# KwonGihyun/TweedieMix

Hardware: AMD Instinct MI355X
Metric: denoise steps/sec @ SDXL 1024^2 K=3 concepts (fusion phase); images/sec at 1/2/4/8 GPUs (higher is better)
Workload: dtype bf16

## Files before the change

tweediemix_amd/csrc/attention.hip:

```cpp
#include "common.h"
#include <type_traits>
#include <stdlib.h>

namespace {

#ifndef TMIX_ATTN_ABL
#define TMIX_ATTN_ABL 0
#endif
constexpr int AABL = TMIX_ATTN_ABL;

typedef __attribute__((ext_vector_type(8))) __bf16 frag_ab;
typedef __attribute__((ext_vector_type(2))) __bf16 bf16x2_t;

constexpr int QB = 128;
constexpr int KB = 64;
constexpr int TILE = KB * 64 * 2;
constexpr int STAGE = 2 * TILE;

struct AttnParams {
    const bf16_t* Q; int64_t ldq, strideQ;
    const bf16_t* K; int64_t ldk, strideK;
    const bf16_t* Vt; int64_t ldvt, strideVt;
    bf16_t* O; int64_t ldo, strideO;
    int B, H, Sq, Skv, nq;
    float scale_log2e;
    unsigned long long* prof; int prof_detail;
    unsigned char* O8; int64_t ldo8; unsigned char* Sc; int64_t ldSc;
    int n_full, lsplit, tpp; float* ws; unsigned* tickets;
};

__device__ __forceinline__ void glds16(const void* gsrc, char* lds_dst) {
    __builtin_amdgcn_global_load_lds((const __attribute__((address_space(1))) void*)gsrc,
                                     (__attribute__((address_space(3))) void*)lds_dst, 16, 0, 0);
}

template <int N> __device__ __forceinline__ void wait_vmcnt() { asm volatile("s_waitcnt vmcnt(%0)" ::"n"(N) : "memory"); }

__device__ __forceinline__ float xor16_max(float x) {
    auto r = __builtin_amdgcn_permlane16_swap(__float_as_uint(x), __float_as_uint(x), false, false);
    return fmaxf(__uint_as_float(r[0]), __uint_as_float(r[1]));
}
__device__ __forceinline__ float xor32_max(float x) {
    auto r = __builtin_amdgcn_permlane32_swap(__float_as_uint(x), __float_as_uint(x), false, false);
    return fmaxf(__uint_as_float(r[0]), __uint_as_float(r[1]));
}
__device__ __forceinline__ float xor16_sum(float x) {
    auto r = __builtin_amdgcn_permlane16_swap(__float_as_uint(x), __float_as_uint(x), false, false);
    return __uint_as_float(r[0]) + __uint_as_float(r[1]);
}
__device__ __forceinline__ float xor32_sum(float x) {
    auto r = __builtin_amdgcn_permlane32_swap(__float_as_uint(x), __float_as_uint(x), false, false);
    return __uint_as_float(r[0]) + __uint_as_float(r[1]);
}

__device__ __forceinline__ void store_row_f8(const AttnParams& p, int64_t row, int h, int fg, const float (&v)[4][4], bool ok) {
#pragma unroll
    for (int blk = 0; blk < 2; ++blk) {
        float f[8], am = 0.f;
#pragma unroll
        for (int k = 0; k < 8; ++k) {
            f[k] = (float)(__bf16)v[2 * blk + (k >> 2)][k & 3];
            am = fmaxf(am, fabsf(f[k]));
        }
        am = xor16_max(am); am = xor32_max(am);
        const int e = e8m0_for_amax(am);
        const float inv = exp2_neg_int(e);
        int q0 = __builtin_amdgcn_cvt_pk_fp8_f32(f[0] * inv, f[1] * inv, 0, false); q0 = __builtin_amdgcn_cvt_pk_fp8_f32(f[2] * inv, f[3] * inv, q0, true);
        int q1 = __builtin_amdgcn_cvt_pk_fp8_f32(f[4] * inv, f[5] * inv, 0, false); q1 = __builtin_amdgcn_cvt_pk_fp8_f32(f[6] * inv, f[7] * inv, q1, true);
        if (ok) {
            unsigned char* dst = p.O8 + row * p.ldo8 + h * 64 + blk * 32 + fg * 4;
            *(int*)dst = q0; *(int*)(dst + 16) = q1;
            if (fg == 0) p.Sc[(int64_t)(h * 2 + blk) * p.ldSc + row] = (unsigned char)(e + 127);
        }
    }
}

constexpr int SPLIT_MAX = 4;
constexpr int SPLIT_VEC = 9;
__device__ __forceinline__ void st_coherent(f32x4* dst, f32x4 v) { asm volatile("global_store_dwordx4 %0, %1, off sc1" :: "v"(dst), "v"(v) : "memory"); }
__device__ __forceinline__ f32x4 ld_coherent(const f32x4* src) { f32x4 v; asm volatile("global_load_dwordx4 %0, %1, off sc1" : "=v"(v) : "v"(src) : "memory"); return v; }

__device__ __forceinline__ uint32_t pk_bf16(float a, float b) {
    bf16x2_t v = {(__bf16)a, (__bf16)b};
    return *(uint32_t*)&v;
}

constexpr int NSP = 4;
constexpr int SMEM_P = NSP * STAGE;

__global__ void __launch_bounds__(256, 2) attn_fwd_pipe_kernel(const AttnParams p) {
#ifndef TMIX_NO_KERNARG_TOUCH
    kernarg_touch<(int)sizeof(AttnParams)>();
#endif
    constexpr int LOADS = 4;
    constexpr int NR = 2;
    extern __shared__ __attribute__((aligned(16))) char smem[];
    const int tid = threadIdx.x, lane = tid & 63;
    const int w = __builtin_amdgcn_readfirstlane(tid >> 6);
    const int fr = lane & 15, fg = lane >> 4;
    const bool prof_on = p.prof != nullptr && tid == 0;
    unsigned long long pt0 = 0, pt1 = 0, pt2 = 0;
    if (prof_on) pt0 = prof_enter(p.prof, blockIdx.x == 0, p.prof_detail);

    int bid, part = 0;
    if ((int)blockIdx.x < p.n_full) bid = xcd_remap(blockIdx.x, p.n_full);
    else {
        const int j = (int)blockIdx.x - p.n_full, k = j >> 3, n_tail8 = ((int)gridDim.x - p.n_full) >> (3 + p.lsplit);
        bid = p.n_full + (j & 7) * n_tail8 + (k >> p.lsplit);
        part = k & ((1 << p.lsplit) - 1);
    }
    const bool split = (int)blockIdx.x >= p.n_full;
    const int bh = bid / p.nq, qt = bid - bh * p.nq;
    const int b = bh / p.H, h = bh - b * p.H;
    const int q0 = qt * QB + w * 32;
    const int key0 = split ? part * p.tpp * KB : 0;
    const int skv = split ? p.tpp * KB : p.Skv;
    const bf16_t* Qb = p.Q + (int64_t)b * p.strideQ + h * 64;
    const bf16_t* Kb = p.K + (int64_t)b * p.strideK + h * 64 + (int64_t)key0 * p.ldk;
    const bf16_t* Vb = p.Vt + (int64_t)b * p.strideVt + (int64_t)h * 64 * p.ldvt + key0;

    const int lrow = lane >> 3;
    const int schunk = ((lane & 7) ^ lrow) * 8;
    int krow[NR], voff[NR];
    const int ldk = (int)p.ldk, ldvt = (int)p.ldvt;
#pragma unroll
    for (int r = 0; r < NR; ++r) {
        const int rho = (r * 4 + w) * 8 + lrow;
        const int f = rho >> 4, i = rho & 15;
        krow[r] = 32 * (f >> 1) + 8 * (i >> 2) + 4 * (f & 1) + (i & 3);
        voff[r] = rho * ldvt;
    }
    const int nt = (skv + KB - 1) / KB;
    const int vlim = ldvt - 8 - key0;
    auto stage = [&](int t) {
        char* sK = smem + (t & (NSP - 1)) * STAGE;
        char* sV = sK + TILE;
        const int kv0 = t * KB;
        int c = kv0 + schunk; if (c > vlim) c = vlim;
#pragma unroll
        for (int r = 0; r < NR; ++r) {
            const int off = (r * 4 + w) * 1024;
            int key = kv0 + krow[r]; if (key > skv - 1) key = skv - 1;
            glds16(Kb + (unsigned)(key * ldk + schunk), sK + off);
            glds16(Vb + (unsigned)(voff[r] + c), sV + off);
        }
    };
#pragma unroll
    for (int t = 0; t < NSP - 1; ++t)
        if (t < nt) stage(t);

    frag_ab qf[2][2];
#pragma unroll
    for (int qi = 0; qi < 2; ++qi) {
        int q = q0 + qi * 16 + fr; if (q > p.Sq - 1) q = p.Sq - 1;
#pragma unroll
        for (int ds = 0; ds < 2; ++ds) {
            const frag_ab raw = *(const frag_ab*)(Qb + (int64_t)q * p.ldq + ds * 32 + fg * 8);
#pragma unroll
            for (int j = 0; j < 8; ++j) qf[qi][ds][j] = (__bf16)((float)raw[j] * p.scale_log2e);
        }
    }

    f32x4 o[4][2];
#pragma unroll
    for (int i = 0; i < 4; ++i) { o[i][0] = (f32x4){0.f, 0.f, 0.f, 0.f}; o[i][1] = (f32x4){0.f, 0.f, 0.f, 0.f}; }
    constexpr float THR = 8.0f;
    f32x4 negm[2] = {{0.f, 0.f, 0.f, 0.f}, {0.f, 0.f, 0.f, 0.f}};
    f32x4 lacc[2] = {{0.f, 0.f, 0.f, 0.f}, {0.f, 0.f, 0.f, 0.f}};
    frag_ab ones;
#pragma unroll
    for (int j = 0; j < 8; ++j) ones[j] = (__bf16)1.0f;
    bool first = true;

    frag_ab kf[2][4];
    frag_ab vf[2][4];
    uint32_t pb[2][2][4];
    const int swk0 = ((0 * 4 + fg) ^ (fr & 7)) << 4, swk1 = ((1 * 4 + fg) ^ (fr & 7)) << 4;
    auto read_k = [&](int t) {
        const char* sK = smem + (t & (NSP - 1)) * STAGE;
#pragma unroll
        for (int f = 0; f < 4; ++f) kf[0][f] = *(const frag_ab*)(sK + (f * 16 + fr) * 128 + swk0);
    };

    auto half1 = [&](int t, f32x4 (&sc)[4][2], f32x4 (&sp)[4][2], auto cur_tag, auto prev_tag) {
        constexpr bool CUR = decltype(cur_tag)::value, PREV = decltype(prev_tag)::value;
        const char* sV = smem + ((t - 1) & (NSP - 1)) * STAGE + TILE;
        const char* sKc = smem + (t & (NSP - 1)) * STAGE;
#pragma unroll
        for (int n = 0; n < 16; ++n) {
            const int dh = n >> 3, f = (n >> 1) & 3, qi = n & 1;
            if constexpr (CUR) {
                if constexpr (AABL & 4) { if (dh == 0) sc[f][qi] = negm[qi]; asm volatile("" :: "v"(kf[dh][f])); }
                else sc[f][qi] = __builtin_amdgcn_mfma_f32_16x16x32_bf16(kf[dh][f], qf[qi][dh], dh ? sc[f][qi] : negm[qi], 0, 0, 0);
            }
// ... 110 lines not shown
    } else {
        half1(nt, sB, sA, F_{}, T_{});
        asm volatile("s_waitcnt lgkmcnt(0)" ::: "memory");
        half2(nt, sB, F_{}, T_{}, F_{});
    }

    if (prof_on) pt2 = prof_now();
    if (split) {
        const int nparts = 1 << p.lsplit, itail = bid - p.n_full;
        f32x4* wsb = (f32x4*)p.ws + ((int64_t)(itail * nparts) * 4 + w) * (SPLIT_VEC * 64) + lane;
        {
            f32x4* dst = wsb + (int64_t)part * 4 * (SPLIT_VEC * 64);
#pragma unroll
            for (int i = 0; i < 8; ++i) st_coherent(dst + i * 64, o[i >> 1][i & 1]);
            st_coherent(dst + 8 * 64, (f32x4){negm[0][0], negm[1][0], lacc[0][0], lacc[1][0]});
        }
        asm volatile("s_waitcnt vmcnt(0)" ::: "memory");
        __syncthreads();
        unsigned* flag = (unsigned*)smem;
        if (tid == 0) {
            const unsigned old = __hip_atomic_fetch_add(p.tickets + itail, 1u, __ATOMIC_RELAXED, __HIP_MEMORY_SCOPE_AGENT);
            const bool last = old == (unsigned)(nparts - 1);
            if (last) __hip_atomic_store(p.tickets + itail, 0u, __ATOMIC_RELAXED, __HIP_MEMORY_SCOPE_AGENT);
            *flag = last;
        }
        __syncthreads();
        if (!*flag) { if (prof_on) prof_leave(p.prof, p.prof_detail, pt0, pt1, pt2); return; }
        f32x4 st[SPLIT_MAX];
#pragma unroll
        for (int r = 0; r < SPLIT_MAX; ++r) if (r < nparts) st[r] = ld_coherent(wsb + (int64_t)r * 4 * (SPLIT_VEC * 64) + 8 * 64);
        asm volatile("s_waitcnt vmcnt(0)" ::: "memory");
        float m0 = -INFINITY, m1 = -INFINITY;
#pragma unroll
        for (int r = 0; r < SPLIT_MAX; ++r) if (r < nparts) { asm volatile("" : "+v"(st[r])); m0 = fmaxf(m0, -st[r][0]); m1 = fmaxf(m1, -st[r][1]); }
#pragma unroll
        for (int i = 0; i < 4; ++i) { o[i][0] = (f32x4){0.f, 0.f, 0.f, 0.f}; o[i][1] = (f32x4){0.f, 0.f, 0.f, 0.f}; }
        float l0 = 0.f, l1 = 0.f;
#pragma unroll
        for (int r = 0; r < SPLIT_MAX; ++r) {
            if (r >= nparts) break;
            f32x4 v[8];
#pragma unroll
            for (int i = 0; i < 8; ++i) v[i] = ld_coherent(wsb + (int64_t)r * 4 * (SPLIT_VEC * 64) + i * 64);
            asm volatile("s_waitcnt vmcnt(0)" ::: "memory");
            const float w0 = __builtin_amdgcn_exp2f(-st[r][0] - m0), w1 = __builtin_amdgcn_exp2f(-st[r][1] - m1);
#pragma unroll
            for (int i = 0; i < 8; ++i) { asm volatile("" : "+v"(v[i])); o[i >> 1][i & 1] += v[i] * ((i & 1) ? w1 : w0); }
            l0 += st[r][2] * w0; l1 += st[r][3] * w1;
        }
        lacc[0][0] = l0; lacc[1][0] = l1;
    }
    if (p.O8) {
#pragma unroll
        for (int qi = 0; qi < 2; ++qi) {
            const int q = q0 + qi * 16 + fr;
            const float inv = 1.0f / lacc[qi][0];
            float v[4][4];
#pragma unroll
            for (int df = 0; df < 4; ++df)
#pragma unroll
                for (int r = 0; r < 4; ++r) v[df][r] = o[df][qi][r] * inv;
            store_row_f8(p, (int64_t)b * p.Sq + min(q, p.Sq - 1), h, fg, v, q < p.Sq);
        }
        if (prof_on) prof_leave(p.prof, p.prof_detail, pt0, pt1, pt2);
        return;
    }
    bf16_t* Ob = p.O + (int64_t)b * p.strideO + h * 64;
#pragma unroll
    for (int qi = 0; qi < 2; ++qi) {
        const int q = q0 + qi * 16 + fr;
        if (q >= p.Sq) continue;
        const float inv = 1.0f / lacc[qi][0];
#pragma unroll
        for (int df = 0; df < 4; ++df) {
            uint2 v;
            v.x = pk_bf16(o[df][qi][0] * inv, o[df][qi][1] * inv);
            v.y = pk_bf16(o[df][qi][2] * inv, o[df][qi][3] * inv);
            *(uint2*)(Ob + (int64_t)q * p.ldo + df * 16 + fg * 4) = v;
        }
    }
    if (prof_on) prof_leave(p.prof, p.prof_detail, pt0, pt1, pt2);
}

constexpr int SK_MAX = 96;
constexpr int SQW = 64;

__global__ void __launch_bounds__(320, 2) attn_small_kernel(const AttnParams p) {
#ifndef TMIX_NO_KERNARG_TOUCH
    kernarg_touch<(int)sizeof(AttnParams)>();
#endif
    const int tid = threadIdx.x, lane = tid & 63;
    const int w = __builtin_amdgcn_readfirstlane(tid >> 6);
    const int fr = lane & 15, fg = lane >> 4;
    const bool prof_on = p.prof != nullptr && tid == 0;
    unsigned long long pt0 = 0, pt1 = 0;
    if (prof_on) pt0 = prof_enter(p.prof, blockIdx.x == 0, p.prof_detail);
    const int bid = xcd_remap(blockIdx.x, gridDim.x);
    const int gw = bid * (int)(blockDim.x >> 6) + w;
    const int bh = gw / p.nq, qt = gw - bh * p.nq;
    const int b = bh / p.H, h = bh - b * p.H;
    const int q0 = qt * SQW;
    if (b >= p.B) {
        if (prof_on) prof_leave(p.prof, p.prof_detail, pt0, pt0, pt0);
        return;
    }
    const bf16_t* Qb = p.Q + (int64_t)b * p.strideQ + h * 64;
    const bf16_t* Kb = p.K + (int64_t)b * p.strideK + h * 64;
    const bf16_t* Vb = p.Vt + (int64_t)b * p.strideVt + (int64_t)h * 64 * p.ldvt;
    bf16_t* Ob = p.O + (int64_t)b * p.strideO + h * 64;
    const int ldvt = (int)p.ldvt;

    frag_ab kf[6][2], vf[3][4];
#pragma unroll
    for (int f = 0; f < 6; ++f) {
        int key = 32 * (f >> 1) + 8 * (fr >> 2) + 4 * (f & 1) + (fr & 3); if (key > p.Skv - 1) key = p.Skv - 1;
#pragma unroll
        for (int ds = 0; ds < 2; ++ds) kf[f][ds] = *(const frag_ab*)(Kb + (int64_t)key * p.ldk + ds * 32 + fg * 8);
    }
#pragma unroll
    for (int ps = 0; ps < 3; ++ps) {
        int c = 32 * ps + fg * 8; if (c > ldvt - 8) c = ldvt - 8;
#pragma unroll
        for (int df = 0; df < 4; ++df) vf[ps][df] = *(const frag_ab*)(Vb + (df * 16 + fr) * ldvt + c);
    }
    frag_ab ones;
#pragma unroll
    for (int j = 0; j < 8; ++j) ones[j] = (__bf16)1.0f;
    frag_ab qraw[SQW / 32][2][2];
#pragma unroll
    for (int blk = 0; blk < SQW / 32; ++blk)
#pragma unroll
        for (int qi = 0; qi < 2; ++qi) {
            int q = q0 + blk * 32 + qi * 16 + fr; if (q > p.Sq - 1) q = p.Sq - 1;
#pragma unroll
            for (int ds = 0; ds < 2; ++ds) qraw[blk][qi][ds] = *(const frag_ab*)(Qb + (int64_t)q * p.ldq + ds * 32 + fg * 8);
        }
    if (prof_on) pt1 = prof_now();

#pragma unroll
    for (int blk = 0; blk < SQW / 32; ++blk) {
        const int qb = q0 + blk * 32;
        if (qb >= p.Sq) break;
        frag_ab qf[2][2];
#pragma unroll
        for (int qi = 0; qi < 2; ++qi) {
#pragma unroll
            for (int ds = 0; ds < 2; ++ds) {
                const frag_ab raw = qraw[blk][qi][ds];
#pragma unroll
                for (int j = 0; j < 8; ++j) qf[qi][ds][j] = (__bf16)((float)raw[j] * p.scale_log2e);
            }
        }
        f32x4 s[6][2];
        const f32x4 zero = {0.f, 0.f, 0.f, 0.f};
#pragma unroll
        for (int f = 0; f < 6; ++f)
#pragma unroll
            for (int qi = 0; qi < 2; ++qi) {
                s[f][qi] = __builtin_amdgcn_mfma_f32_16x16x32_bf16(kf[f][0], qf[qi][0], zero, 0, 0, 0);
                s[f][qi] = __builtin_amdgcn_mfma_f32_16x16x32_bf16(kf[f][1], qf[qi][1], s[f][qi], 0, 0, 0);
            }
        uint32_t pb[2][3][4];
        f32x4 o[4][2], lacc[2];
#pragma unroll
        for (int qi = 0; qi < 2; ++qi) {
            float m = -INFINITY;
#pragma unroll
            for (int f = 0; f < 6; ++f)
#pragma unroll
                for (int r = 0; r < 4; ++r) {
                    if (32 * (f >> 1) + 8 * fg + 4 * (f & 1) + r >= p.Skv) s[f][qi][r] = -INFINITY;
                    m = fmaxf(m, s[f][qi][r]);
                }
            m = xor32_max(xor16_max(m));
#pragma unroll
            for (int f = 0; f < 6; ++f)
#pragma unroll
                for (int r = 0; r < 4; ++r) s[f][qi][r] = __builtin_amdgcn_exp2f(s[f][qi][r] - m);
#pragma unroll
            for (int ps = 0; ps < 3; ++ps) {
                pb[qi][ps][0] = pk_bf16(s[2 * ps][qi][0], s[2 * ps][qi][1]);
                pb[qi][ps][1] = pk_bf16(s[2 * ps][qi][2], s[2 * ps][qi][3]);
                pb[qi][ps][2] = pk_bf16(s[2 * ps + 1][qi][0], s[2 * ps + 1][qi][1]);
                pb[qi][ps][3] = pk_bf16(s[2 * ps + 1][qi][2], s[2 * ps + 1][qi][3]);
            }
            lacc[qi] = zero;
#pragma unroll
            for (int df = 0; df < 4; ++df) o[df][qi] = zero;
        }
#pragma unroll
        for (int ps = 0; ps < 3; ++ps) {
            frag_ab p0, p1;
            __builtin_memcpy(&p0, pb[0][ps], 16);
            __builtin_memcpy(&p1, pb[1][ps], 16);
            lacc[0] = __builtin_amdgcn_mfma_f32_16x16x32_bf16(ones, p0, lacc[0], 0, 0, 0);
            lacc[1] = __builtin_amdgcn_mfma_f32_16x16x32_bf16(ones, p1, lacc[1], 0, 0, 0);
#pragma unroll
            for (int df = 0; df < 4; ++df) {
                o[df][0] = __builtin_amdgcn_mfma_f32_16x16x32_bf16(vf[ps][df], p0, o[df][0], 0, 0, 0);
                o[df][1] = __builtin_amdgcn_mfma_f32_16x16x32_bf16(vf[ps][df], p1, o[df][1], 0, 0, 0);
            }
        }
#pragma unroll
        for (int qi = 0; qi < 2; ++qi) {
            const int q = qb + qi * 16 + fr;
            const float inv = 1.0f / lacc[qi][0];
            if (p.O8) {
                float v[4][4];
#pragma unroll
                for (int df = 0; df < 4; ++df)
#pragma unroll
                    for (int r = 0; r < 4; ++r) v[df][r] = o[df][qi][r] * inv;
                store_row_f8(p, (int64_t)b * p.Sq + min(q, p.Sq - 1), h, fg, v, q < p.Sq);
                continue;
            }
            if (q >= p.Sq) continue;
#pragma unroll
            for (int df = 0; df < 4; ++df) {
                uint2 v;
                v.x = pk_bf16(o[df][qi][0] * inv, o[df][qi][1] * inv);
                v.y = pk_bf16(o[df][qi][2] * inv, o[df][qi][3] * inv);
                *(uint2*)(Ob + (int64_t)q * p.ldo + df * 16 + fg * 4) = v;
            }
        }
    }
    if (prof_on) prof_leave(p.prof, p.prof_detail, pt0, pt1, pt1);
}

}

struct AttnSplit { int n_full, lsplit, tpp, n_tail; int64_t ws_bytes; };
static bool attn_split_device_ok() {
    static int ok = -1;
    if (ok < 0) {
        int dev = 0; hipDeviceProp_t prop;
        ok = (hipGetDevice(&dev) == hipSuccess && hipGetDeviceProperties(&prop, dev) == hipSuccess && prop.multiProcessorCount * 2 == 512) ? 1 : 0;
    }
    return ok == 1;
}
static bool attn_split_plan(int B, int H, int Sq, int Skv, AttnSplit& sp) {
    constexpr int SLOTS = 512, TICKET_BYTES = 4096;
    if (Skv <= SK_MAX || (Skv % KB) || tmix_env(TMIX_ENV_ATTN_NO_SPLIT)) return false;
    const int64_t items = (int64_t)((Sq + QB - 1) / QB) * B * H;
    const int nt = Skv / KB;
    const int r = (int)(items % SLOTS);
    if (items <= SLOTS || r == 0 || (r & 7) || (SLOTS % r)) return false;
    int split = SLOTS / r, lsplit = 0;
    if (split > SPLIT_MAX) split = SPLIT_MAX;
    while ((1 << lsplit) < split) ++lsplit;
    if ((1 << lsplit) != split || (nt % split) || nt / split < 2 || r > TICKET_BYTES / 4) return false;
    sp.n_full = (int)(items - r); sp.lsplit = lsplit; sp.tpp = nt / split; sp.n_tail = r;
    sp.ws_bytes = TICKET_BYTES + (int64_t)r * split * 4 * SPLIT_VEC * 64 * 16;
    return true;
}

extern "C" int64_t tmix_attn_split_ws_bytes(int B, int H, int Sq, int Skv) {
    AttnSplit sp;
    if (B <= 0 || H <= 0 || Sq <= 0 || Skv <= 0) return 0;
    return attn_split_plan(B, H, Sq, Skv, sp) ? sp.ws_bytes : 0;
}

static int attn_entry(const void* Q, int64_t ldq, int64_t strideQ, const void* K, int64_t ldk, int64_t strideK,
                      const void* Vt, int64_t ldvt, int64_t strideVt, void* O, int64_t ldo, int64_t strideO,
                      void* O8, int64_t ldo8, void* Sc, int64_t ldSc,
                      int B, int H, int Sq, int Skv, float scale, void* stream, void* ws = nullptr, int64_t ws_bytes = 0) {
    if (!Q || !K || !Vt || (!O && !O8)) TMIX_FAIL(TMIX_EINVAL, "attn: null pointer");
    if (O8) {
        if (!Sc || (ldo8 % 4) || ldo8 < (int64_t)H * 64 || ldSc < (int64_t)B * Sq || (((uintptr_t)O8) & 3))
            TMIX_FAIL(TMIX_EINVAL, "attn_f8: needs the scale array [H*2][ldSc >= B*Sq] and 4-byte aligned e4m3 rows of ldo8 >= H*64 bytes");
        O = (void*)Q; ldo = 4; strideO = 4;
    }
    if (B <= 0 || H <= 0 || Sq <= 0 || Skv <= 0) TMIX_FAIL(TMIX_ESHAPE, "attn: empty problem B=%d H=%d Sq=%d Skv=%d", B, H, Sq, Skv);
    if ((int64_t)Skv * ldk >= (1ll << 31) || 64 * ldvt >= (1ll << 31)) TMIX_FAIL(TMIX_ESHAPE, "attn: per-head K/V extent exceeds 32-bit offsets");
    if ((ldq % 8) || (ldk % 8) || (ldvt % 8) || (ldo % 4) || (strideQ % 8) || (strideK % 8) || (strideVt % 8) || (strideO % 4))
        TMIX_FAIL(TMIX_EALIGN, "attn: leading dims / strides must keep 16-byte (Q,K,Vt) / 8-byte (O) alignment");
    if (ldvt < ((Skv + 7) / 8) * 8) TMIX_FAIL(TMIX_ESHAPE, "attn: ldvt=%lld < Skv rounded up to 8", (long long)ldvt);
    if (!aligned16(Q) || !aligned16(K) || !aligned16(Vt) || (((uintptr_t)O) & 7)) TMIX_FAIL(TMIX_EALIGN, "attn: pointer alignment");
    static bool attr_set = false;
    if (!attr_set) {
        hipError_t e = hipFuncSetAttribute((const void*)attn_fwd_pipe_kernel, hipFuncAttributeMaxDynamicSharedMemorySize, SMEM_P);
        if (e != hipSuccess) TMIX_FAIL((int)e, "hipFuncSetAttribute: %s", hipGetErrorString(e));
        attr_set = true;
    }
    AttnParams p;
    p.Q = (const bf16_t*)Q; p.ldq = ldq; p.strideQ = strideQ;
    p.K = (const bf16_t*)K; p.ldk = ldk; p.strideK = strideK;
    p.Vt = (const bf16_t*)Vt; p.ldvt = ldvt; p.strideVt = strideVt;
    p.O = (bf16_t*)O; p.ldo = ldo; p.strideO = strideO;
    p.O8 = (unsigned char*)O8; p.ldo8 = ldo8; p.Sc = (unsigned char*)Sc; p.ldSc = ldSc;
    p.B = B; p.H = H; p.Sq = Sq; p.Skv = Skv; p.nq = (Sq + QB - 1) / QB;
    p.scale_log2e = scale * 1.4426950408889634f;
    p.prof = tmix_prof_take(&p.prof_detail);
    if (Skv <= SK_MAX && !tmix_env(TMIX_ENV_ATTN_GENERAL)) {
        p.nq = (Sq + SQW - 1) / SQW;
        const int64_t waves = (int64_t)p.nq * B * H;
        const int64_t w4 = (waves + 3) / 4, w5 = (waves + 4) / 5;
        const int64_t c4 = ((w4 + 255) / 256) * 4, c5 = ((w5 + 255) / 256) * 5;
        const int nwv = c5 < c4 ? 5 : 4;
        const int64_t nws = nwv == 5 ? w5 : w4;
        if (nws > 0x7fffffff) TMIX_FAIL(TMIX_ESHAPE, "attn: grid too large");
        attn_small_kernel<<<dim3((unsigned)nws), nwv * 64, 0, (hipStream_t)stream>>>(p);
        TMIX_LAUNCH_CHECK();
        return TMIX_OK;
    }
    int64_t nwg = (int64_t)p.nq * B * H;
    if (nwg > 0x7fffffff) TMIX_FAIL(TMIX_ESHAPE, "attn: grid too large");
    p.n_full = (int)nwg; p.lsplit = 0; p.tpp = 0; p.ws = nullptr; p.tickets = nullptr;
    AttnSplit sp;
    if (ws && attn_split_device_ok() && attn_split_plan(B, H, Sq, Skv, sp)) {
        if ((((uintptr_t)ws) & 15) || ws_bytes < sp.ws_bytes)
            TMIX_FAIL(TMIX_EINVAL, "attn: the key-split workspace needs %lld bytes (tmix_attn_split_ws_bytes), 16-byte aligned; got %lld", (long long)sp.ws_bytes, (long long)ws_bytes);
        p.n_full = sp.n_full; p.lsplit = sp.lsplit; p.tpp = sp.tpp;
        p.tickets = (unsigned*)ws; p.ws = (float*)((char*)ws + 4096);
        nwg = (int64_t)sp.n_full + ((int64_t)sp.n_tail << sp.lsplit);
    }
    attn_fwd_pipe_kernel<<<dim3((unsigned)nwg), 256, SMEM_P, (hipStream_t)stream>>>(p);
    if (p.tickets) {
        hipError_t e_ = hipGetLastError();
        if (e_ != hipSuccess) {
            (void)hipMemsetAsync(p.tickets, 0, 4096, (hipStream_t)stream);
            TMIX_FAIL((int)e_, "%s:%d launch failed: %s", __FILE__, __LINE__, hipGetErrorString(e_));
        }
        return TMIX_OK;
    }
    TMIX_LAUNCH_CHECK();
    return TMIX_OK;
}

extern "C" int tmix_attn_fwd(const void* Q, int64_t ldq, int64_t strideQ, const void* K, int64_t ldk, int64_t strideK,
                             const void* Vt, int64_t ldvt, int64_t strideVt, void* O, int64_t ldo, int64_t strideO,
                             int B, int H, int Sq, int Skv, float scale, void* stream) {
    return attn_entry(Q, ldq, strideQ, K, ldk, strideK, Vt, ldvt, strideVt, O, ldo, strideO, nullptr, 0, nullptr, 0, B, H, Sq, Skv, scale, stream);
}

extern "C" int tmix_attn_fwd_f8(const void* Q, int64_t ldq, int64_t strideQ, const void* K, int64_t ldk, int64_t strideK,
                                const void* Vt, int64_t ldvt, int64_t strideVt, void* O8, int64_t ldo8, void* scales, int64_t ldScale,
                                int B, int H, int Sq, int Skv, float scale, void* stream) {
    if (!O8) TMIX_FAIL(TMIX_EINVAL, "attn_f8: null output");
    return attn_entry(Q, ldq, strideQ, K, ldk, strideK, Vt, ldvt, strideVt, nullptr, 0, 0, O8, ldo8, scales, ldScale, B, H, Sq, Skv, scale, stream);
}

extern "C" int tmix_attn_fwd_ws(const void* Q, int64_t ldq, int64_t strideQ, const void* K, int64_t ldk, int64_t strideK,
                                const void* Vt, int64_t ldvt, int64_t strideVt, void* O, int64_t ldo, int64_t strideO,
                                int B, int H, int Sq, int Skv, float scale, void* ws, int64_t ws_bytes, void* stream) {
    return attn_entry(Q, ldq, strideQ, K, ldk, strideK, Vt, ldvt, strideVt, O, ldo, strideO, nullptr, 0, nullptr, 0, B, H, Sq, Skv, scale, stream, ws, ws_bytes);
}

extern "C" int tmix_attn_fwd_f8_ws(const void* Q, int64_t ldq, int64_t strideQ, const void* K, int64_t ldk, int64_t strideK,
                                   const void* Vt, int64_t ldvt, int64_t strideVt, void* O8, int64_t ldo8, void* scales, int64_t ldScale,
                                   int B, int H, int Sq, int Skv, float scale, void* ws, int64_t ws_bytes, void* stream) {
    if (!O8) TMIX_FAIL(TMIX_EINVAL, "attn_f8: null output");
    return attn_entry(Q, ldq, strideQ, K, ldk, strideK, Vt, ldvt, strideVt, nullptr, 0, 0, O8, ldo8, scales, ldScale, B, H, Sq, Skv, scale, stream, ws, ws_bytes);
}
```

tweediemix_amd/csrc/capi.cpp:

```cpp
#include "common.h"
#include <stdlib.h>
#include <string.h>

static thread_local char g_err[512] = "";

void tmix_set_error(const char* fmt, ...) {
    va_list ap;
    va_start(ap, fmt);
    vsnprintf(g_err, sizeof(g_err), fmt, ap);
    va_end(ap);
}

static thread_local TmixProf g_prof = {nullptr, 0, 0, 0};
TmixProf& tmix_prof_state() { return g_prof; }

extern "C" int tmix_prof_begin(uint64_t* slots, int capacity, int detail) {
    if (!slots || capacity < 1 || (((uintptr_t)slots) & 7)) TMIX_FAIL(TMIX_EINVAL, "prof_begin: need an 8-byte aligned device buffer of capacity >= 1 slots");
    g_prof.buf = (unsigned long long*)slots; g_prof.cap = capacity; g_prof.next = 0; g_prof.detail = detail ? 1 : 0;
    return TMIX_OK;
}
extern "C" int tmix_prof_end(void) {
    const int used = g_prof.next;
    g_prof.buf = nullptr; g_prof.cap = 0; g_prof.next = 0; g_prof.detail = 0;
    return used;
}

static thread_local const char* g_pf_ptr = nullptr;
static thread_local long long g_pf_bytes = 0;
void tmix_prefetch_take(const char** ptr, long long* bytes) {
    *ptr = g_pf_bytes > 0 ? g_pf_ptr : nullptr; *bytes = g_pf_bytes > 0 ? g_pf_bytes : 0;
    g_pf_ptr = nullptr; g_pf_bytes = 0;
}
extern "C" int tmix_gemm_prefetch_next(const void* next_weights, int64_t bytes, void* ) {
    if (bytes > (1ll << 31)) TMIX_FAIL(TMIX_ESHAPE, "gemm_prefetch_next: %lld bytes (at most 2 GiB)", (long long)bytes);
    g_pf_ptr = (next_weights && bytes > 0) ? (const char*)next_weights : nullptr;
    g_pf_bytes = g_pf_ptr ? bytes : 0;
    return TMIX_OK;
}

static const char* const g_env_names[TMIX_ENV_COUNT] = {"TMIX_GN_NO_SMALL", "TMIX_ATTN_NO_SPLIT", "TMIX_ATTN_GENERAL", "TMIX_NARROW_EPILOGUE"};
static int g_env[TMIX_ENV_COUNT];
static bool g_env_read = false;
extern "C" void tmix_env_refresh(void) {
    for (int i = 0; i < TMIX_ENV_COUNT; ++i) g_env[i] = getenv(g_env_names[i]) != nullptr;
    g_env_read = true;
}
bool tmix_env(int which) {
    if (!g_env_read) tmix_env_refresh();
    return g_env[which] != 0;
}

extern "C" int tmix_version(void) { return TMIX_VERSION; }
extern "C" const char* tmix_last_error_string(void) { return g_err; }

extern "C" int tmix_check_device(void) {
    int dev = 0;
    hipError_t e = hipGetDevice(&dev);
    if (e != hipSuccess) TMIX_FAIL((int)e, "hipGetDevice: %s", hipGetErrorString(e));
    hipDeviceProp_t p;
    e = hipGetDeviceProperties(&p, dev);
    if (e != hipSuccess) TMIX_FAIL((int)e, "hipGetDeviceProperties: %s", hipGetErrorString(e));
    if (strncmp(p.gcnArchName, "gfx950", 6) != 0) TMIX_FAIL(TMIX_EARCH, "device arch %s is not gfx950", p.gcnArchName);
    return TMIX_OK;
}
```

tweediemix_amd/csrc/common.h:

```cpp
#pragma once
#include <hip/hip_runtime.h>
#include <hip/hip_fp16.h>
#include <stdint.h>
#include <stdio.h>
#include <stdarg.h>
#include "../../include/tmix.h"

typedef uint16_t bf16_t;
typedef __attribute__((ext_vector_type(8))) short  bf16x8;
typedef __attribute__((ext_vector_type(4))) float  f32x4;
typedef __attribute__((ext_vector_type(16))) float f32x16;

__device__ __forceinline__ float bf2f(bf16_t v) { return __uint_as_float(((uint32_t)v) << 16); }
typedef __bf16 bf16x2_hw __attribute__((ext_vector_type(2)));
typedef float f32x2_hw __attribute__((ext_vector_type(2)));
__device__ __forceinline__ uint32_t pack_bf2(float lo, float hi) {
#if defined(TMIX_ABL_SW_BF16)
    uint32_t a = __float_as_uint(lo), b = __float_as_uint(hi);
    a = ((a & 0x7fffffffu) > 0x7f800000u) ? ((a >> 16) | 0x40u) : ((a + 0x7fffu + ((a >> 16) & 1u)) >> 16);
    b = ((b & 0x7fffffffu) > 0x7f800000u) ? ((b >> 16) | 0x40u) : ((b + 0x7fffu + ((b >> 16) & 1u)) >> 16);
    return (a & 0xffffu) | (b << 16);
#else
    const f32x2_hw f = {lo, hi};
    const bf16x2_hw b = __builtin_convertvector(f, bf16x2_hw);
    return __builtin_bit_cast(uint32_t, b);
#endif
}
__device__ __forceinline__ bf16_t f2bf(float f) { return (bf16_t)(pack_bf2(f, f) & 0xffffu); }
__device__ __forceinline__ float silu_f(float x) { return x / (1.0f + __expf(-x)); }
__device__ __forceinline__ float gelu_erf_f(float x) {
    const float a = fminf(fabsf(x), 5.5f);
    float p = -1.921234625e-06f;
    p = __builtin_fmaf(p, a, 6.328849712e-05f);
    p = __builtin_fmaf(p, a, -9.434208502e-04f);
    p = __builtin_fmaf(p, a, 8.556272268e-03f);
    p = __builtin_fmaf(p, a, -5.405228293e-02f);
    p = __builtin_fmaf(p, a, -4.583817849e-01f);
    p = __builtin_fmaf(p, a, -1.151278331e+00f);
    p = __builtin_fmaf(p, a, -9.999938561e-01f);
    const float e = __builtin_amdgcn_exp2f(p);
    return x * (x < 0.f ? e : 1.0f - e);
}

__device__ __forceinline__ int e8m0_for_amax(float amax) {
    if (!(amax > 0.f)) return 0;
    const unsigned bits = __float_as_uint(amax * (1.0f / 448.0f));
    int e = (int)((bits >> 23) & 0xff) - 127 + ((bits & 0x7fffff) ? 1 : 0);
    return e < -127 ? -127 : (e > 127 ? 127 : e);
}
__device__ __forceinline__ float exp2_neg_int(int e) { return e >= 127 ? __uint_as_float(0x00400000u) : __uint_as_float((unsigned)(127 - e) << 23); }

void tmix_set_error(const char* fmt, ...);

enum { TMIX_ENV_GN_NO_SMALL = 0, TMIX_ENV_ATTN_NO_SPLIT, TMIX_ENV_ATTN_GENERAL, TMIX_ENV_NARROW_EPILOGUE, TMIX_ENV_COUNT };
bool tmix_env(int which);
#define TMIX_FAIL(code, ...) do { tmix_set_error(__VA_ARGS__); return (code); } while (0)
#define TMIX_LAUNCH_CHECK() do { hipError_t e_ = hipGetLastError(); if (e_ != hipSuccess) { \
    tmix_set_error("%s:%d launch failed: %s", __FILE__, __LINE__, hipGetErrorString(e_)); return (int)e_; } } while (0)

static inline bool aligned16(const void* p) { return (((uintptr_t)p) & 15u) == 0; }

struct TmixProf { unsigned long long* buf; int cap, next, detail; };
TmixProf& tmix_prof_state();
static inline unsigned long long* tmix_prof_take(int* detail = nullptr) {
    TmixProf& st = tmix_prof_state();
    if (detail) *detail = st.detail;
    if (!st.buf || st.next >= st.cap) return nullptr;
    return st.buf + 8 * (size_t)(st.next++);
}
void tmix_prefetch_take(const char** ptr, long long* bytes);
__device__ __forceinline__ unsigned long long prof_now() { return __builtin_amdgcn_s_memrealtime(); }
__device__ __forceinline__ unsigned long long prof_enter(unsigned long long* slot, bool first, int detail) {
    const unsigned long long t = prof_now();
    if (detail) atomicMin(slot, t);
    else if (first) __hip_atomic_store(slot, t, __ATOMIC_RELAXED, __HIP_MEMORY_SCOPE_AGENT);
    return t;
}
__device__ __forceinline__ void prof_leave(unsigned long long* slot, int detail, unsigned long long t0, unsigned long long t1, unsigned long long t2) {
    if (detail) {
        const unsigned long long t3 = prof_now();
        atomicMax(slot + 1, t3);
        atomicAdd(slot + 2, t1 - t0); atomicAdd(slot + 3, t2 - t0); atomicAdd(slot + 4, t3 - t0); atomicAdd(slot + 5, 1ull);
    } else {
        const unsigned lin = (blockIdx.z * gridDim.y + blockIdx.y) * gridDim.x + blockIdx.x, total = gridDim.x * gridDim.y * gridDim.z;
        if (lin + 32 >= total) __hip_atomic_store(slot + 1, prof_now(), __ATOMIC_RELAXED, __HIP_MEMORY_SCOPE_AGENT);
    }
}

template <int BYTES> __device__ __forceinline__ void kernarg_touch() {
    const auto ka = __builtin_amdgcn_kernarg_segment_ptr();
    constexpr int LINES = (BYTES + 63) / 64;
    static_assert(LINES >= 1 && LINES <= 8, "kernarg block larger than expected");
    unsigned t0, t1, t2, t3, t4, t5, t6, t7;
    asm volatile("s_load_dword %0, %8, 0x0\n\t"
                 "s_load_dword %1, %8, %9\n\t"
                 "s_load_dword %2, %8, %10\n\t"
                 "s_load_dword %3, %8, %11\n\t"
                 "s_load_dword %4, %8, %12\n\t"
                 "s_load_dword %5, %8, %13\n\t"
                 "s_load_dword %6, %8, %14\n\t"
                 "s_load_dword %7, %8, %15\n\t"
                 "s_waitcnt lgkmcnt(0)"
                 : "=&s"(t0), "=&s"(t1), "=&s"(t2), "=&s"(t3), "=&s"(t4), "=&s"(t5), "=&s"(t6), "=&s"(t7)
                 : "s"(ka), "n"(LINES > 1 ? 0x40 : 0), "n"(LINES > 2 ? 0x80 : 0), "n"(LINES > 3 ? 0xc0 : 0), "n"(LINES > 4 ? 0x100 : 0),
                   "n"(LINES > 5 ? 0x140 : 0), "n"(LINES > 6 ? 0x180 : 0), "n"(LINES > 7 ? 0x1c0 : 0)
                 : "memory");
}

__device__ __forceinline__ int xcd_remap(int bid, int nwg) {
    const int q = nwg >> 3, r = nwg & 7;
    const int xcd = bid & 7, idx = bid >> 3;
    const int base = (xcd < r) ? xcd * (q + 1) : r * (q + 1) + (xcd - r) * q;
    return base + idx;
}
__device__ __forceinline__ void xcd_remap_grid(int& bid, int& by) {
    const int gx = gridDim.x, gy = gridDim.y;
    if (gy == 1) { bid = xcd_remap(blockIdx.x, gx); by = blockIdx.y; return; }
    const int lg = xcd_remap(blockIdx.y * gx + blockIdx.x, gx * gy);
    by = lg / gx; bid = lg - by * gx;
}
```

Measured before the change: 31.25.

## Add 32x32 MFMA attention kernel and launch split tail separately

Adds a new flash-attention kernel built on 32x32x16 bf16 MFMA instructions, with a different LDS swizzle and softmax pipeline, and makes it the default path when Skv and Sq are tile-aligned. The key-split tail blocks are now launched as a separate pipe-kernel grid offset by wg0, so the full tiles go through the new kernel. The aim is to cut register shuffling and raise matrix-unit throughput per wave compared with the 16x16 layout. Thread-safe env and attribute initialisation (atomics, call_once, per-device cache) is also added. The cost is an extra kernel launch when splitting and a large new code path that needs checking for correctness and register pressure.

New measurement: 31.68, median of 6. 1.01x the previous value.

```diff
diff --git a/tweediemix_amd/csrc/attention.hip b/tweediemix_amd/csrc/attention.hip
--- a/tweediemix_amd/csrc/attention.hip
+++ b/tweediemix_amd/csrc/attention.hip
@@ -1,5 +1,7 @@
 #include "common.h"
 #include <type_traits>
+#include <atomic>
+#include <mutex>
 #include <stdlib.h>
 
 namespace {
@@ -27,6 +29,7 @@
     unsigned long long* prof; int prof_detail;
     unsigned char* O8; int64_t ldo8; unsigned char* Sc; int64_t ldSc;
     int n_full, lsplit, tpp; float* ws; unsigned* tickets;
+    int wg0;
 };
 
 __device__ __forceinline__ void glds16(const void* gsrc, char* lds_dst) {
@@ -103,13 +106,14 @@
     if (prof_on) pt0 = prof_enter(p.prof, blockIdx.x == 0, p.prof_detail);
 
     int bid, part = 0;
-    if ((int)blockIdx.x < p.n_full) bid = xcd_remap(blockIdx.x, p.n_full);
+    const int lb = (int)blockIdx.x + p.wg0, lgrid = (int)gridDim.x + p.wg0;
+    if (lb < p.n_full) bid = xcd_remap(lb, p.n_full);
     else {
-        const int j = (int)blockIdx.x - p.n_full, k = j >> 3, n_tail8 = ((int)gridDim.x - p.n_full) >> (3 + p.lsplit);
+        const int j = lb - p.n_full, k = j >> 3, n_tail8 = (lgrid - p.n_full) >> (3 + p.lsplit);
         bid = p.n_full + (j & 7) * n_tail8 + (k >> p.lsplit);
         part = k & ((1 << p.lsplit) - 1);
     }
-    const bool split = (int)blockIdx.x >= p.n_full;
+    const bool split = lb >= p.n_full;
     const int bh = bid / p.nq, qt = bid - bh * p.nq;
     const int b = bh / p.H, h = bh - b * p.H;
     const int q0 = qt * QB + w * 32;
@@ -386,6 +390,272 @@
     if (prof_on) prof_leave(p.prof, p.prof_detail, pt0, pt1, pt2);
 }
 
+constexpr int NW64 = 4;
+#ifndef TMIX_ATTN_W64_NQB
+#define TMIX_ATTN_W64_NQB 1
+#endif
+constexpr int NQB64 = TMIX_ATTN_W64_NQB;
+constexpr int QB64 = NW64 * 32 * NQB64;
+
+__device__ __forceinline__ f32x16 mfma32(const frag_ab& a, const frag_ab& b, const f32x16& c) {
+    return __builtin_amdgcn_mfma_f32_32x32x16_bf16(a, b, c, 0, 0, 0);
+}
+
+__global__ void __launch_bounds__(256, 3 - NQB64) __attribute__((amdgpu_waves_per_eu(3 - NQB64, 3 - NQB64))) attn_w64_kernel(const AttnParams p) {
+#ifndef TMIX_NO_KERNARG_TOUCH
+    kernarg_touch<(int)sizeof(AttnParams)>();
+#endif
+    constexpr int LOADS = 4;
+    constexpr int NR = 2;
+    extern __shared__ __attribute__((aligned(16))) char smem[];
+    const int tid = threadIdx.x, lane = tid & 63;
+    const int w = __builtin_amdgcn_readfirstlane(tid >> 6);
+    const int r32 = lane & 31, hh = lane >> 5;
+    const bool prof_on = p.prof != nullptr && tid == 0;
+    unsigned long long pt0 = 0, pt1 = 0, pt2 = 0;
+    if (prof_on) pt0 = prof_enter(p.prof, blockIdx.x == 0, p.prof_detail);
+
+    const int bid = xcd_remap(blockIdx.x, gridDim.x);
+    const int bh = bid / p.nq, qt = bid - bh * p.nq;
+    const int b = bh / p.H, h = bh - b * p.H;
+    const int q0 = qt * QB64 + w * 32 * NQB64;
+    const bf16_t* Qb = p.Q + (int64_t)b * p.strideQ + h * 64;
+    const bf16_t* Kb = p.K + (int64_t)b * p.strideK + h * 64;
+    const bf16_t* Vb = p.Vt + (int64_t)b * p.strideVt + (int64_t)h * 64 * p.ldvt;
+
+    frag_ab qraw[NQB64][4];
+#pragma unroll
+    for (int qb = 0; qb < NQB64; ++qb) {
+        int q = q0 + qb * 32 + r32; if (q > p.Sq - 1) q = p.Sq - 1;
+#pragma unroll
+        for (int ds = 0; ds < 4; ++ds) qraw[qb][ds] = *(const frag_ab*)(Qb + (int64_t)q * p.ldq + ds * 16 + hh * 8);
+    }
+
+    const int lrow = lane >> 3;
+    const int schunk = ((lane & 7) ^ lrow) * 8;
+    int krow[NR], voff[NR];
+    const int ldk = (int)p.ldk, ldvt = (int)p.ldvt;
+#pragma unroll
+    for (int r = 0; r < NR; ++r) {
+        const int rho = (r * NW64 + w) * 8 + lrow;
+        const int x = rho & 31;
+        krow[r] = (rho & 32) + ((x & 19) | ((x >> 1) & 4) | ((x << 1) & 8));
+        voff[r] = rho * ldvt;
+    }
+    const int nt = p.Skv / KB;
+    auto stage = [&](int t) {
+        char* sK = smem + (t & (NSP - 1)) * STAGE;
+        char* sV = sK + TILE;
+        const int kv0 = t * KB;
+#pragma unroll
+        for (int r = 0; r < NR; ++r) {
+            const int off = (r * NW64 + w) * 1024;
+            glds16(Kb + (unsigned)((kv0 + krow[r]) * ldk + schunk), sK + off);
+            glds16(Vb + (unsigned)(voff[r] + kv0 + schunk), sV + off);
+        }
+    };
+#pragma unroll
+    for (int t = 0; t < NSP - 1; ++t)
+        if (t < nt) stage(t);
+
+    frag_ab qf[NQB64][4];
+#pragma unroll
+    for (int qb = 0; qb < NQB64; ++qb)
+#pragma unroll
+        for (int ds = 0; ds < 4; ++ds)
+#pragma unroll
+            for (int j = 0; j < 8; ++j) qf[qb][ds][j] = (__bf16)((float)qraw[qb][ds][j] * p.scale_log2e);
+
+    f32x16 o[2][NQB64], lacc[NQB64], negm[NQB64];
+#pragma unroll
+    for (int qb = 0; qb < NQB64; ++qb)
+#pragma unroll
+        for (int i = 0; i < 16; ++i) { o[0][qb][i] = 0.f; o[1][qb][i] = 0.f; lacc[qb][i] = 0.f; negm[qb][i] = 0.f; }
+    constexpr float THR = 8.0f;
+    frag_ab ones;
+#pragma unroll
+    for (int j = 0; j < 8; ++j) ones[j] = (__bf16)1.0f;
+    bool first = true;
+
+    frag_ab kf[2][4];
+    frag_ab vf[2][2][2];
+    uint32_t pb[2][NQB64][2][4];
+    auto kaddr = [&](int kb, int ds) { return (kb * 32 + r32) * 128 + (((2 * ds + hh) ^ (r32 & 7)) << 4); };
+    auto read_k = [&](int t) {
+        const char* sK = smem + (t & (NSP - 1)) * STAGE;
+#pragma unroll
+        for (int n = 0; n < 4; ++n) kf[0][n] = *(const frag_ab*)(sK + kaddr(0, n));
+    };
+    auto pack_word = [&](const f32x16 (&sp)[2][NQB64], int kb, int wd) {
+        const int qb = wd >> 3, s = (wd >> 2) & 1, k = wd & 3;
+        const float e0 = __builtin_amdgcn_exp2f(sp[kb][qb][8 * s + 2 * k]);
+        const float e1 = __builtin_amdgcn_exp2f(sp[kb][qb][8 * s + 2 * k + 1]);
+        pb[kb][qb][s][k] = pk_bf16(e0, e1);
+        asm volatile("" : "+v"(pb[kb][qb][s][k]));
+    };
+    auto read_v = [&](const char* sV, int kb, int m) {
+        const int s = m >> 1, db = m & 1, d = db * 32 + r32;
+        vf[kb][s][db] = *(const frag_ab*)(sV + d * 128 + (((4 * kb + 2 * s + hh) ^ (r32 & 7)) << 4));
+    };
+    auto pv_mfma = [&](int kb, int n) {
+        const int s = n / (3 * NQB64), m = n % (3 * NQB64);
+        if (m < NQB64) {
+            frag_ab pp; __builtin_memcpy(&pp, pb[kb][m][s], 16);
+            lacc[m] = mfma32(ones, pp, lacc[m]);
+        } else {
+            const int db = (m - NQB64) / NQB64, qb = (m - NQB64) % NQB64;
+            frag_ab pp; __builtin_memcpy(&pp, pb[kb][qb][s], 16);
+            o[db][qb] = mfma32(vf[kb][s][db], pp, o[db][qb]);
+        }
+    };
+
+    auto tile = [&](int t, f32x16 (&sc)[2][NQB64], f32x16 (&sp)[2][NQB64], auto cur_tag, auto prev_tag) {
+        constexpr bool CUR = decltype(cur_tag)::value, PREV = decltype(prev_tag)::value;
+        const char* sV = smem + ((t - 1) & (NSP - 1)) * STAGE + TILE;
+        const char* sKc = smem + (t & (NSP - 1)) * STAGE;
+#pragma unroll
+        for (int n = 0; n < 8 * NQB64; ++n) {
+            if constexpr (CUR) {
+                const int kb = n / (4 * NQB64), qb = (n >> 2) % NQB64, ds = n & 3;
+                sc[kb][qb] = mfma32(kf[kb][ds], qf[qb][ds], ds ? sc[kb][qb] : negm[qb]);
+            }
+            __builtin_amdgcn_sched_barrier(0);
+            if constexpr (CUR) { if (n < 4) kf[1][n] = *(const frag_ab*)(sKc + kaddr(1, n)); }
+            if constexpr (PREV) {
+                pack_word(sp, 0, n);
+                if (n >= 4 && n < 8) read_v(sV, 0, n - 4);
+            }
+            __builtin_amdgcn_sched_barrier(0);
+        }
+#pragma unroll
+        for (int n = 0; n < 6 * NQB64; ++n) {
+            if constexpr (PREV) pv_mfma(0, n);
+            __builtin_amdgcn_sched_barrier(0);
+            if constexpr (PREV) {
+#pragma unroll
+                for (int wd = 0; wd < 8 * NQB64; ++wd) if (((wd * 3) >> 2) == n) pack_word(sp, 1, wd);
+                if (n >= 2 && n < 6) read_v(sV, 1, n - 2);
+            }
+            __builtin_amdgcn_sched_barrier(0);
+        }
+        if constexpr (CUR) {
+            asm volatile("s_waitcnt lgkmcnt(0)" ::: "memory");
+            if (t + 2 < nt) wait_vmcnt<LOADS>(); else wait_vmcnt<0>();
+            __builtin_amdgcn_sched_barrier(0);
+            __builtin_amdgcn_s_barrier();
+            __builtin_amdgcn_sched_barrier(0);
+            asm volatile("" ::: "memory");
+            if (t + 3 < nt) stage(t + 3);
+        }
+        int im = 0x80000000;
+        const char* sKn = smem + ((t + 1) & (NSP - 1)) * STAGE;
+#pragma unroll
+        for (int n = 0; n < 6 * NQB64; ++n) {
+            if constexpr (PREV) pv_mfma(1, n);
+            __builtin_amdgcn_sched_barrier(0);
+            if constexpr (CUR) {
+                if (n < 4 * NQB64) {
+                    const int kb = n / (2 * NQB64), qb = (n >> 1) % NQB64, i0 = (n & 1) * 8;
+                    const f32x16& v = sc[kb][qb];
+                    im = max(max(max(im, __float_as_int(v[i0])), max(__float_as_int(v[i0 + 1]), __float_as_int(v[i0 + 2]))),
+                             max(max(__float_as_int(v[i0 + 3]), __float_as_int(v[i0 + 4])), max(max(__float_as_int(v[i0 + 5]), __float_as_int(v[i0 + 6])), __float_as_int(v[i0 + 7]))));
+                }
+                if (n >= 6 * NQB64 - 4) kf[0][n - (6 * NQB64 - 4)] = *(const frag_ab*)(sKn + kaddr(0, n - (6 * NQB64 - 4)));
+            }
+            __builtin_amdgcn_sched_barrier(0);
+        }
+        if constexpr (CUR) {
+            if (first || __any(im > __float_as_int(THR))) {
+#pragma unroll
+                for (int qb = 0; qb < NQB64; ++qb) {
+                    float m0 = sc[0][qb][0];
+#pragma unroll
+                    for (int i = 1; i < 16; ++i) m0 = fmaxf(m0, sc[0][qb][i]);
+#pragma unroll
+                    for (int i = 0; i < 16; ++i) m0 = fmaxf(m0, sc[1][qb][i]);
+                    float delta = xor32_max(m0);
+                    if (!first) delta = fmaxf(delta, 0.f);
+                    const float alpha = first ? 0.f : __builtin_amdgcn_exp2f(-delta);
+                    sc[0][qb] = sc[0][qb] - delta;
+                    sc[1][qb] = sc[1][qb] - delta;
+                    o[0][qb] *= alpha;
+                    o[1][qb] *= alpha;
+                    lacc[qb] *= alpha;
+                    negm[qb] = negm[qb] - delta;
+                }
+                first = false;
+            }
+        }
+    };
+
+    f32x16 sA[2][NQB64], sB[2][NQB64];
+    using T_ = std::true_type; using F_ = std::false_type;
+    if (nt >= NSP - 1) wait_vmcnt<(NSP - 2) * LOADS>(); else if (nt == 2) wait_vmcnt<LOADS>(); else wait_vmcnt<0>();
+    __builtin_amdgcn_s_barrier();
+    asm volatile("" ::: "memory");
+    if (prof_on) pt1 = prof_now();
+    read_k(0);
+    tile(0, sA, sB, T_{}, F_{});
+    int t = 1;
+    for (; t + 1 < nt; t += 2) {
+        tile(t, sB, sA, T_{}, T_{});
+        tile(t + 1, sA, sB, T_{}, T_{});
+    }
+    if (t < nt) {
+        tile(t, sB, sA, T_{}, T_{});
+        tile(t + 1, sA, sB, F_{}, T_{});
+    } else {
+        tile(nt, sB, sA, F_{}, T_{});
+    }
+    if (prof_on) pt2 = prof_now();
+
+    if (p.O8) {
+#pragma unroll
+        for (int qb = 0; qb < NQB64; ++qb) {
+            const int q = q0 + qb * 32 + r32;
+            const float inv = 1.0f / lacc[qb][0];
+            const bool ok = q < p.Sq;
+            const int64_t row = (int64_t)b * p.Sq + min(q, p.Sq - 1);
+#pragma unroll
+            for (int db = 0; db < 2; ++db) {
+                float f[16], am = 0.f;
+#pragma unroll
+                for (int i = 0; i < 16; ++i) { f[i] = (float)(__bf16)(o[db][qb][i] * inv); am = fmaxf(am, fabsf(f[i])); }
+                am = xor32_max(am);
+                const int e = e8m0_for_amax(am);
+                const float sinv = exp2_neg_int(e);
+                unsigned char* dst = p.O8 + row * p.ldo8 + h * 64 + db * 32 + hh * 4;
+#pragma unroll
+                for (int g = 0; g < 4; ++g) {
+                    int qv = __builtin_amdgcn_cvt_pk_fp8_f32(f[4 * g] * sinv, f[4 * g + 1] * sinv, 0, false);
+                    qv = __builtin_amdgcn_cvt_pk_fp8_f32(f[4 * g + 2] * sinv, f[4 * g + 3] * sinv, qv, true);
+                    if (ok) *(int*)(dst + 8 * g) = qv;
+                }
+                if (ok && hh == 0) p.Sc[(int64_t)(h * 2 + db) * p.ldSc + row] = (unsigned char)(e + 127);
+            }
+        }
+        if (prof_on) prof_leave(p.prof, p.prof_detail, pt0, pt1, pt2);
+        return;
+    }
+    bf16_t* Ob = p.O + (int64_t)b * p.strideO + h * 64;
+#pragma unroll
+    for (int qb = 0; qb < NQB64; ++qb) {
+        const int q = q0 + qb * 32 + r32;
+        if (q >= p.Sq) continue;
+        const float inv = 1.0f / lacc[qb][0];
+#pragma unroll
+        for (int db = 0; db < 2; ++db)
+#pragma unroll
+            for (int g = 0; g < 4; ++g) {
+                uint2 v;
+                v.x = pk_bf16(o[db][qb][4 * g] * inv, o[db][qb][4 * g + 1] * inv);
+                v.y = pk_bf16(o[db][qb][4 * g + 2] * inv, o[db][qb][4 * g + 3] * inv);
+                *(uint2*)(Ob + (int64_t)q * p.ldo + db * 32 + 8 * g + 4 * hh) = v;
+            }
+    }
+    if (prof_on) prof_leave(p.prof, p.prof_detail, pt0, pt1, pt2);
+}
+
 constexpr int SK_MAX = 96;
 constexpr int SQW = 64;
 
@@ -535,12 +805,16 @@
 
 struct AttnSplit { int n_full, lsplit, tpp, n_tail; int64_t ws_bytes; };
 static bool attn_split_device_ok() {
-    static int ok = -1;
-    if (ok < 0) {
-        int dev = 0; hipDeviceProp_t prop;
-        ok = (hipGetDevice(&dev) == hipSuccess && hipGetDeviceProperties(&prop, dev) == hipSuccess && prop.multiProcessorCount * 2 == 512) ? 1 : 0;
-    }
-    return ok == 1;
+    static std::atomic<signed char> ok[64];
+    int dev = 0;
+    if (hipGetDevice(&dev) != hipSuccess || dev < 0 || dev >= 64) return false;
+    signed char v = ok[dev].load(std::memory_order_relaxed);
+    if (v == 0) {
+        hipDeviceProp_t prop;
+        v = (hipGetDeviceProperties(&prop, dev) == hipSuccess && prop.multiProcessorCount * 2 == 512) ? 1 : -1;
+        ok[dev].store(v, std::memory_order_relaxed);
+    }
+    return v == 1;
 }
 static bool attn_split_plan(int B, int H, int Sq, int Skv, AttnSplit& sp) {
     constexpr int SLOTS = 512, TICKET_BYTES = 4096;
@@ -580,12 +854,13 @@
         TMIX_FAIL(TMIX_EALIGN, "attn: leading dims / strides must keep 16-byte (Q,K,Vt) / 8-byte (O) alignment");
     if (ldvt < ((Skv + 7) / 8) * 8) TMIX_FAIL(TMIX_ESHAPE, "attn: ldvt=%lld < Skv rounded up to 8", (long long)ldvt);
     if (!aligned16(Q) || !aligned16(K) || !aligned16(Vt) || (((uintptr_t)O) & 7)) TMIX_FAIL(TMIX_EALIGN, "attn: pointer alignment");
-    static bool attr_set = false;
-    if (!attr_set) {
-        hipError_t e = hipFuncSetAttribute((const void*)attn_fwd_pipe_kernel, hipFuncAttributeMaxDynamicSharedMemorySize, SMEM_P);
-        if (e != hipSuccess) TMIX_FAIL((int)e, "hipFuncSetAttribute: %s", hipGetErrorString(e));
-        attr_set = true;
-    }
+    static std::once_flag attr_once;
+    static hipError_t attr_err = hipSuccess;
+    std::call_once(attr_once, [] {
+        attr_err = hipFuncSetAttribute((const void*)attn_fwd_pipe_kernel, hipFuncAttributeMaxDynamicSharedMemorySize, SMEM_P);
+        if (attr_err == hipSuccess) attr_err = hipFuncSetAttribute((const void*)attn_w64_kernel, hipFuncAttributeMaxDynamicSharedMemorySize, SMEM_P);
+    });
+    if (attr_err != hipSuccess) TMIX_FAIL((int)attr_err, "hipFuncSetAttribute: %s", hipGetErrorString(attr_err));
     AttnParams p;
     p.Q = (const bf16_t*)Q; p.ldq = ldq; p.strideQ = strideQ;
     p.K = (const bf16_t*)K; p.ldk = ldk; p.strideK = strideK;
@@ -607,18 +882,34 @@
         TMIX_LAUNCH_CHECK();
         return TMIX_OK;
     }
-    int64_t nwg = (int64_t)p.nq * B * H;
-    if (nwg > 0x7fffffff) TMIX_FAIL(TMIX_ESHAPE, "attn: grid too large");
-    p.n_full = (int)nwg; p.lsplit = 0; p.tpp = 0; p.ws = nullptr; p.tickets = nullptr;
+    p.wg0 = 0; p.n_full = 0; p.lsplit = 0; p.tpp = 0; p.ws = nullptr; p.tickets = nullptr;
     AttnSplit sp;
-    if (ws && attn_split_device_ok() && attn_split_plan(B, H, Sq, Skv, sp)) {
-        if ((((uintptr_t)ws) & 15) || ws_bytes < sp.ws_bytes)
-            TMIX_FAIL(TMIX_EINVAL, "attn: the key-split workspace needs %lld bytes (tmix_attn_split_ws_bytes), 16-byte aligned; got %lld", (long long)sp.ws_bytes, (long long)ws_bytes);
-        p.n_full = sp.n_full; p.lsplit = sp.lsplit; p.tpp = sp.tpp;
+    const bool split = ws && attn_split_device_ok() && attn_split_plan(B, H, Sq, Skv, sp);
+    if (split && ((((uintptr_t)ws) & 15) || ws_bytes < sp.ws_bytes))
+        TMIX_FAIL(TMIX_EINVAL, "attn: the key-split workspace needs %lld bytes (tmix_attn_split_ws_bytes), 16-byte aligned; got %lld", (long long)sp.ws_bytes, (long long)ws_bytes);
+    if (!tmix_env(TMIX_ENV_ATTN_PIPE) && Skv % KB == 0 && Sq % (32 * NQB64) == 0) {
+        p.nq = (Sq + QB64 - 1) / QB64;
+        const int64_t nwg = (int64_t)p.nq * B * H;
+        if (nwg > 0x7fffffff) TMIX_FAIL(TMIX_ESHAPE, "attn: grid too large");
+        attn_w64_kernel<<<dim3((unsigned)nwg), NW64 * 64, SMEM_P, (hipStream_t)stream>>>(p);
+        TMIX_LAUNCH_CHECK();
+        if (!split) return TMIX_OK;
+        p.prof = nullptr;
+        p.nq = (Sq + QB - 1) / QB;
+        p.n_full = sp.n_full; p.lsplit = sp.lsplit; p.tpp = sp.tpp; p.wg0 = sp.n_full;
         p.tickets = (unsigned*)ws; p.ws = (float*)((char*)ws + 4096);
-        nwg = (int64_t)sp.n_full + ((int64_t)sp.n_tail << sp.lsplit);
-    }
-    attn_fwd_pipe_kernel<<<dim3((unsigned)nwg), 256, SMEM_P, (hipStream_t)stream>>>(p);
+        attn_fwd_pipe_kernel<<<dim3((unsigned)((int64_t)sp.n_tail << sp.lsplit)), 256, SMEM_P, (hipStream_t)stream>>>(p);
+    } else {
+        int64_t nwg = (int64_t)p.nq * B * H;
+        if (nwg > 0x7fffffff) TMIX_FAIL(TMIX_ESHAPE, "attn: grid too large");
+        p.n_full = (int)nwg;
+        if (split) {
+            p.n_full = sp.n_full; p.lsplit = sp.lsplit; p.tpp = sp.tpp;
+            p.tickets = (unsigned*)ws; p.ws = (float*)((char*)ws + 4096);
+            nwg = (int64_t)sp.n_full + ((int64_t)sp.n_tail << sp.lsplit);
+        }
+        attn_fwd_pipe_kernel<<<dim3((unsigned)nwg), 256, SMEM_P, (hipStream_t)stream>>>(p);
+    }
     if (p.tickets) {
         hipError_t e_ = hipGetLastError();
         if (e_ != hipSuccess) {
diff --git a/tweediemix_amd/csrc/capi.cpp b/tweediemix_amd/csrc/capi.cpp
--- a/tweediemix_amd/csrc/capi.cpp
+++ b/tweediemix_amd/csrc/capi.cpp
@@ -1,6 +1,8 @@
 #include "common.h"
 #include <stdlib.h>
 #include <string.h>
+#include <atomic>
+#include <mutex>
 
 static thread_local char g_err[512] = "";
 
@@ -38,16 +40,16 @@
     return TMIX_OK;
 }
 
-static const char* const g_env_names[TMIX_ENV_COUNT] = {"TMIX_GN_NO_SMALL", "TMIX_ATTN_NO_SPLIT", "TMIX_ATTN_GENERAL", "TMIX_NARROW_EPILOGUE"};
-static int g_env[TMIX_ENV_COUNT];
-static bool g_env_read = false;
+static const char* const g_env_names[TMIX_ENV_COUNT] = {"TMIX_GN_NO_SMALL", "TMIX_ATTN_NO_SPLIT", "TMIX_ATTN_GENERAL", "TMIX_NARROW_EPILOGUE",
+                                                          "TMIX_ATTN_PIPE"};
+static std::atomic<bool> g_env[TMIX_ENV_COUNT];
+static std::once_flag g_env_once;
 extern "C" void tmix_env_refresh(void) {
-    for (int i = 0; i < TMIX_ENV_COUNT; ++i) g_env[i] = getenv(g_env_names[i]) != nullptr;
-    g_env_read = true;
+    for (int i = 0; i < TMIX_ENV_COUNT; ++i) g_env[i].store(getenv(g_env_names[i]) != nullptr, std::memory_order_relaxed);
 }
 bool tmix_env(int which) {
-    if (!g_env_read) tmix_env_refresh();
-    return g_env[which] != 0;
+    std::call_once(g_env_once, tmix_env_refresh);
+    return g_env[which].load(std::memory_order_relaxed);
 }
 
 extern "C" int tmix_version(void) { return TMIX_VERSION; }
diff --git a/tweediemix_amd/csrc/common.h b/tweediemix_amd/csrc/common.h
--- a/tweediemix_amd/csrc/common.h
+++ b/tweediemix_amd/csrc/common.h
@@ -52,7 +52,7 @@
 
 void tmix_set_error(const char* fmt, ...);
 
-enum { TMIX_ENV_GN_NO_SMALL = 0, TMIX_ENV_ATTN_NO_SPLIT, TMIX_ENV_ATTN_GENERAL, TMIX_ENV_NARROW_EPILOGUE, TMIX_ENV_COUNT };
+enum { TMIX_ENV_GN_NO_SMALL = 0, TMIX_ENV_ATTN_NO_SPLIT, TMIX_ENV_ATTN_GENERAL, TMIX_ENV_NARROW_EPILOGUE, TMIX_ENV_ATTN_PIPE, TMIX_ENV_COUNT };
 bool tmix_env(int which);
 #define TMIX_FAIL(code, ...) do { tmix_set_error(__VA_ARGS__); return (code); } while (0)
 #define TMIX_LAUNCH_CHECK() do { hipError_t e_ = hipGetLastError(); if (e_ != hipSuccess) { \
```
